# amirkdv/biseqt

Measured on AMD Instinct MI355X. Metric: GCUPS (DP cell updates/s) banded local align, higher is better.
Workload: dtype i16

## Files before the change

biseqt_amd/batch.py:

```python
import ctypes as C

import numpy as np

from . import _pwlib as W
from .sequence import Sequence

RESULT_DTYPE = np.dtype([('score', '<f8'), ('opt_i', '<i4'), ('opt_j', '<i4'),
                         ('origin_idx', '<i4'), ('mutant_idx', '<i4'),
                         ('tx_len', '<i4'), ('status', '<i4')])
assert RESULT_DTYPE.itemsize == 32
SUMMARY_DTYPE = np.dtype([(f, '<i4') for f in ('n_match', 'n_subst', 'n_ins', 'n_del', 'n_gaps', 'first_match', 'last_match',
                                               'head_origin', 'head_mutant', 'tail_origin', 'tail_mutant', 'flags')])
assert SUMMARY_DTYPE.itemsize == 48
CIGAR_EXTENDED, CIGAR_CLASSIC = W.PW_CIGAR_EXTENDED, W.PW_CIGAR_CLASSIC
CIGAR_OPS = 'MIDNSHP=X'
_CIGAR_FORMS = {'extended': CIGAR_EXTENDED, 'classic': CIGAR_CLASSIC}
SITE_DTYPE = np.dtype([('depth', '<u4'), ('call', 'u1'), ('ref', 'u1'), ('flags', '<u2')])
assert SITE_DTYPE.itemsize == 8
POLISH_STATS_DTYPE = np.dtype([(f, '<u4') for f in ('kept', 'substituted', 'deleted', 'inserted')])
assert POLISH_STATS_DTYPE.itemsize == 16
_SIDES = {'origin': W.PW_SIDE_ORIGIN, 'mutant': W.PW_SIDE_MUTANT, 'both': W.PW_SIDE_BOTH}
_CIGAR_LETTERS = ({'M': '=', 'S': 'X', 'I': 'I', 'D': 'D'}, {'M': 'M', 'S': 'M', 'I': 'I', 'D': 'D'})


# ... 742 lines not shown

def transcript_of_cigar(s):
    import re
    if not re.fullmatch(r'(?:[0-9]+[A-Za-z=])*', s):
        raise ValueError('not a CIGAR string: %r' % (s,))
    back = {'=': 'M', 'X': 'S', 'I': 'I', 'D': 'D'}
    out = []
    for n, op in re.findall(r'([0-9]+)([A-Za-z=])', s):
        if op not in back:
            raise ValueError('CIGAR op %r has no transcript letter (only the extended form =, X, I, D has)' % (op,))
        out.append(back[op] * int(n))
    return ''.join(out)


def plan_only(shapes, alnmode=W.STD_MODE, alntype=W.GLOBAL, alphabet_len=4, subst_scores=None, match_score=1, mismatch_score=0,
              go_score=0, ge_score=0, flags=0, ramp_free=False, stamp_group=False, lds_feed=False, pair_keys=False):
    lib = W.load()
    L = alphabet_len
    if subst_scores is None:
        subst_scores = [[match_score if i == j else mismatch_score for i in range(L)] for j in range(L)]
    S = np.ascontiguousarray(np.asarray(subst_scores, dtype=np.float64).reshape(L, L))
    sc = W.pw_scoring(alnmode, alntype, L, S.ctypes.data_as(C.POINTER(C.c_double)), float(go_score), float(ge_score))
    pairs = (W.pw_pair * max(len(shapes), 1))()
    off = 0
    for k, sh in enumerate(shapes):
        X, Y = int(sh[0]), int(sh[1])
        dmin, dmax = (int(sh[2]), int(sh[3])) if len(sh) > 2 else (0, 0)
        oo = off
        off += (X + 15) // 16 * 16 + 16
        mo = off
        off += (Y + 15) // 16 * 16 + 16
        pairs[k] = W.pw_pair(oo, mo, X, Y, dmin, dmax)
    name = C.create_string_buffer(128)
    info = (C.c_int32 * 8)()
    if lib.pw_plan_only(C.byref(sc), len(shapes), pairs, max(off, 16), flags, name, 128, info) != 0:
        raise RuntimeError('pw_plan_only failed: ' + W.last_error())
    out = dict(kernel=name.value.decode(), score_dtype='f64' if info[0] else 'i32', scale_shift=info[1], one_wavefront=info[2],
                workgroup=info[3], tiled=info[4], strips=info[5], packed_rule=info[6], matrix=bool(info[7] & 1))
    if ramp_free:
        out['ramp_free'] = bool(info[7] & 2)
    if stamp_group:
        out['stamp_group'] = 4 if info[7] & 4 else 1
    if lds_feed:
        out['lds_feed'] = bool(info[7] & 8)
    if pair_keys:
        out['pair_keys'] = bool(info[7] & 16)
    return out
```

biseqt_amd/csrc/build.py:

```python
import concurrent.futures
import os
import shutil
import subprocess
import sys

HERE = os.path.dirname(os.path.abspath(__file__))
ROOT = os.path.dirname(os.path.dirname(HERE))
OUT_DIR = os.path.join(os.path.dirname(HERE), 'pwlib')
OBJ_DIR = os.path.join(HERE, os.environ.get('PW_OBJ_DIR', '_build'))
SO = os.path.join(OUT_DIR, os.environ.get('PW_SO_NAME', 'pwlib.so'))
HIPCC = os.environ.get('HIPCC', '/opt/rocm/bin/hipcc')
ARCH = 'gfx950'
COMMON = ['--offload-arch=' + ARCH, '-O3', '-std=c++17', '-fPIC', '-ffp-contract=off', '-Wall',
          '-Wno-unused-function'] + os.environ.get('PW_EXTRA_CXXFLAGS', '').split()
BKS = (2, 4, 8, 16, 32)
PACKED_BKS = (4, 8, 12, 16, 20, 24, 28, 32)
PACKED_RULES = (0, 1, 2, 3, 4, 5)
PACKED_MAT_RULES = (0, 1, 2, 3)
FILL16_WAVES = {
    (8, 0, 0): (5, 0), (8, 3, 0): (5, 0),
    (16, 0, 0): (3, 0), (16, 3, 0): (3, 0),
    (8, 0, 1): (3, 0), (8, 3, 1): (3, 0),
}
for _e in filter(None, os.environ.get('PW_FILL16_WAVES_OVERRIDE', '').split(';')):
    _k, _v = _e.split('=')
    FILL16_WAVES[tuple(int(x) for x in _k.split(','))] = tuple(int(x) for x in _v.split(','))
FILL16_UNR = {}
for _e in filter(None, os.environ.get('PW_FILL16_UNR_OVERRIDE', '').split(';')):
    _k, _v = _e.split('=')
    FILL16_UNR[tuple(int(x) for x in _k.split(','))] = int(_v)
TYPES = (('i32', 'int32_t'), ('f64', 'double'))
F64_FLAGS = {'f64': ['-fno-honor-nans'] + os.environ.get('PW_F64_EXTRA_CXXFLAGS', '').split()}
FILL_EXTRA = {('f64', 8): ['-mllvm', '-amdgpu-sched-strategy=max-ilp']}
HASHED_OBJECTS = ('pw_fill16_bk8_r3_mat.o', 'pw_fill16g_bk8_r3_mat.o', 'pw_fill16l_bk8_r3_mat.o', 'pw_fill16p_bk8_r3_mat.o', 'pw_fill16_bk8_r3.o', 'pw_fill16_bk8_r0.o', 'pw_fill_i32_bk8.o', 'pw_fill_f64_bk8.o', 'pw_strip.o')
HEADERS = ['pw_types.h', 'pw_wave.h', 'pw_strip.h', 'pw_plan.h', 'pw_model.h', 'pw_launch.h', 'pw_device.h', 'pw_hip_host.h']


def _jobs():
    jobs = []
    for tn, t in TYPES:
        for bk in BKS:
            obj = os.path.join(OBJ_DIR, 'pw_fill_%s_bk%d.o' % (tn, bk))
            cmd = [HIPCC] + COMMON + F64_FLAGS.get(tn, []) + FILL_EXTRA.get((tn, bk), []) + ['-DPW_T=' + t, '-DPW_TNAME=' + tn, '-DPW_BK=%d' % bk, '-c',
                                      os.path.join(HERE, 'pw_fill_tu.hip'), '-o', obj]
            jobs.append((obj, cmd, [os.path.join(HERE, 'pw_fill_tu.hip')]))
    for tn, t in TYPES:
        obj = os.path.join(OBJ_DIR, 'pw_fill_mw_%s.o' % tn)
        cmd = [HIPCC] + COMMON + F64_FLAGS.get(tn, []) + ['-DPW_T=' + t, '-DPW_TNAME=' + tn, '-c', os.path.join(HERE, 'pw_fill_mw_tu.hip'), '-o', obj]
        jobs.append((obj, cmd, [os.path.join(HERE, 'pw_fill_mw_tu.hip')]))
# ... 10 lines not shown
               os.path.join(HERE, 'pw_fill16_tu.hip'), '-o', obj]
        jobs.append((obj, cmd, [os.path.join(HERE, 'pw_fill16_tu.hip')]))
    obj = os.path.join(OBJ_DIR, 'pw_fill16g_bk8_r3_mat.o')
    occ, occ_seg = FILL16_WAVES.get((8, 3, 1), (0, 0)) if os.environ.get('PW_FILL16_OCCUPANCY', '1') != '0' else (0, 0)
    jobs.append((obj, [HIPCC] + COMMON + ['-mllvm', '-amdgpu-sched-strategy=max-ilp', '-DPW_FILL16_WAVES=%d' % occ,
                                          '-DPW_FILL16_WAVES_SEG=%d' % occ_seg, '-c', os.path.join(HERE, 'pw_fill16g_tu.hip'), '-o', obj],
                 [os.path.join(HERE, 'pw_fill16g_tu.hip')]))
    obj = os.path.join(OBJ_DIR, 'pw_fill16l_bk8_r3_mat.o')
    jobs.append((obj, [HIPCC] + COMMON + ['-mllvm', '-amdgpu-sched-strategy=max-ilp', '-DPW_FILL16_WAVES=%d' % occ,
                                          '-DPW_FILL16_WAVES_SEG=%d' % occ_seg, '-c', os.path.join(HERE, 'pw_fill16l_tu.hip'), '-o', obj],
                 [os.path.join(HERE, 'pw_fill16l_tu.hip')]))
    obj = os.path.join(OBJ_DIR, 'pw_fill16p_bk8_r3_mat.o')
    jobs.append((obj, [HIPCC] + COMMON + ['-mllvm', '-amdgpu-sched-strategy=max-ilp', '-DPW_FILL16_WAVES=%d' % occ,
                                          '-DPW_FILL16_WAVES_SEG=%d' % occ_seg, '-c', os.path.join(HERE, 'pw_fill16p_tu.hip'), '-o', obj],
                 [os.path.join(HERE, 'pw_fill16p_tu.hip')]))
    obj = os.path.join(OBJ_DIR, 'pw_trace.o')
    jobs.append((obj, [HIPCC] + COMMON + ['-c', os.path.join(HERE, 'pw_trace.hip'), '-o', obj],
                 [os.path.join(HERE, 'pw_trace.hip')]))
    obj = os.path.join(OBJ_DIR, 'pw_txsum.o')
    jobs.append((obj, [HIPCC] + COMMON + ['-c', os.path.join(HERE, 'pw_txsum.hip'), '-o', obj],
                 [os.path.join(HERE, 'pw_txsum.hip'), os.path.join(ROOT, 'include', 'pw_txsum.h'), os.path.join(ROOT, 'include', 'pw_batch.h')]))
    obj = os.path.join(OBJ_DIR, 'pw_cigar.o')
    jobs.append((obj, [HIPCC] + COMMON + ['-c', os.path.join(HERE, 'pw_cigar.hip'), '-o', obj],
                 [os.path.join(HERE, 'pw_cigar.hip'), os.path.join(ROOT, 'include', 'pw_cigar.h'), os.path.join(ROOT, 'include', 'pw_batch.h')]))
    obj = os.path.join(OBJ_DIR, 'pw_pileup.o')
    jobs.append((obj, [HIPCC] + COMMON + ['-c', os.path.join(HERE, 'pw_pileup.hip'), '-o', obj],
                 [os.path.join(HERE, 'pw_pileup.hip'), os.path.join(ROOT, 'include', 'pw_pileup.h'), os.path.join(ROOT, 'include', 'pw_batch.h')]))
    obj = os.path.join(OBJ_DIR, 'pw_polish.o')
    jobs.append((obj, [HIPCC] + COMMON + ['-Wno-unused-parameter', '-c', os.path.join(HERE, 'pw_polish.hip'), '-o', obj],
                 [os.path.join(HERE, 'pw_polish.hip'), os.path.join(ROOT, 'include', 'pw_polish.h'), os.path.join(ROOT, 'include', 'pw_pileup.h'),
# ... 119 lines not shown
```

biseqt_amd/csrc/pw_device.h:

```cpp
#ifndef PW_DEVICE_H
#define PW_DEVICE_H

#include <hip/hip_runtime.h>
#include <stdint.h>

#define PW_FN __device__ __forceinline__
#include "pw_wave.h"
#include "pw_launch.h"

namespace pw {

PW_FN uint32_t dev_shl1_in(uint32_t m, bool flag) {
  const uint64_t mask = __builtin_amdgcn_ballot_w64(flag);
  uint32_t r;
  uint64_t cout;
  asm("v_addc_co_u32 %0, %1, %2, %2, %3" : "=v"(r), "=s"(cout) : "v"(m), "s"(mask));
  return r;
}

template <typename T, bool ALWAYS_LDS> PW_FN T dev_tab_read(const T* tab, uint32_t handle, uint32_t off, bool in_lds) {
  typedef __attribute__((address_space(3))) const T lds_T;
  if (ALWAYS_LDS || in_lds) return *(lds_T*)(uintptr_t)(handle + off);
  return *(const T*)((const char*)tab + off);
}
// ... 7 lines not shown
}

typedef uint64_t FeedDwords __attribute__((aligned(4)));
PW_FN uint64_t dev_const_dword2(const uint8_t* base, uint32_t byte_off) {
  typedef const __attribute__((address_space(4))) uint8_t c_u8;
  typedef const __attribute__((address_space(4))) FeedDwords c_fd;
  return *(c_fd*)((c_u8*)base + byte_off + 4u);
}

struct DevFeed {
  PW_FN static uint64_t const_dword2(const uint8_t* base, uint32_t byte_off) { return dev_const_dword2(base, byte_off); }
  PW_FN static uint32_t lds_read32(uint32_t addr) { return *(__attribute__((address_space(3))) const uint32_t*)(uintptr_t)addr; }
  PW_FN static void lds_write32(uint32_t addr, uint32_t v) { *(__attribute__((address_space(3))) uint32_t*)(uintptr_t)addr = v; }
  PW_FN static void lds_write16(uint32_t addr, uint32_t v) { *(__attribute__((address_space(3))) uint16_t*)(uintptr_t)addr = (uint16_t)v; }
  PW_FN static void lds_sync() { __syncthreads(); }
};

struct DevP : DevFeed {
  PW_FN static uint32_t const_dword(const uint8_t* base, int idx) { return dev_const_dword(base, idx); }
  template <typename T, bool A> PW_FN static T tab_read(const T* tab, uint32_t h, uint32_t off, bool in_lds) { return dev_tab_read<T, A>(tab, h, off, in_lds); }
  PW_FN static uint32_t shl1_in(uint32_t m, bool flag) { return dev_shl1_in(m, flag); }
  PW_FN static int lane() { return (int)(threadIdx.x & 63u); }
  PW_FN static int32_t shr1(int32_t v, int32_t old) {
    return __builtin_amdgcn_update_dpp(old, v, 0x138 , 0xf, 0xf, false);
  }
  PW_FN static int32_t shl1(int32_t v, int32_t old) {
    return __builtin_amdgcn_update_dpp(old, v, 0x130 , 0xf, 0xf, false);
  }
  PW_FN static int32_t shr1z(int32_t v) { return __builtin_amdgcn_update_dpp(0, v, 0x138 , 0xf, 0xf, true); }
  PW_FN static int32_t shl1z(int32_t v) { return __builtin_amdgcn_update_dpp(0, v, 0x130 , 0xf, 0xf, true); }
// ... 150 lines not shown
void k_fill16l(const FillParams<int32_t> a) {
  using W = WaveFill16<DevP, BK, SEG, RULE, MAT, 4, true>;
  __shared__ uint32_t ring[2 * W::kRingWords];
  const WaveDesc wd = a.waves[blockIdx.x];
  W w(a, wd);
  w.ring_h = dev_lds_handle(ring);
  w.run();
}

template <int BK, bool SEG, int RULE, bool MAT = false>
__global__ __launch_bounds__(64) PW_FILL_ATTR
__attribute__((amdgpu_waves_per_eu(Fill16Occupancy<BK, SEG, RULE>::lo, Fill16Occupancy<BK, SEG, RULE>::hi)))
void k_fill16p(const FillParams<int32_t> a) {
  using W = WaveFill16<DevP, BK, SEG, RULE, MAT, 4, true, true>;
  __shared__ uint32_t ring[2 * W::kRingWords];
  const WaveDesc wd = a.waves[blockIdx.x];
  W w(a, wd);
  w.ring_h = dev_lds_handle(ring);
  w.run();
}

template <int BK, int RULE, bool MAT = false>
__global__ __launch_bounds__(512) void k_fill16_mw(const FillParams<int32_t> a) {
  const WaveDesc wd = a.waves[blockIdx.x];
  WaveFill16<DevPM, BK, false, RULE, MAT> w(a, wd);
  w.run();
}

constexpr int kTileLanes = PW_TILE_LANES, kTileGhost = PW_TILE_GHOST, kTileCentral = kTileLanes - 2 * kTileGhost;
struct DevPT : DevFeed {
// ... 191 lines not shown
```

biseqt_amd/csrc/pw_launch.h:

```cpp
#ifndef PW_LAUNCH_H
#define PW_LAUNCH_H

#include <hip/hip_runtime_api.h>

#include "pw_plan.h"
#include "pw_types.h"

namespace pw {

hipError_t launch_fill(const FillParams<int32_t>& a, int variant, int bk, int nblocks, hipStream_t st);
hipError_t launch_fill(const FillParams<double>& a, int variant, int bk, int nblocks, hipStream_t st);
hipError_t launch_fill16(const FillParams<int32_t>& a, int bk, int seg, int rule, int mat, int nwaves, hipStream_t st);
hipError_t launch_fill16_mw(const FillParams<int32_t>& a, int bk, int rule, int mat, int nw, int npairs, hipStream_t st);
hipError_t launch_fill16g(const FillParams<int32_t>& a, int nwaves, hipStream_t st);
hipError_t launch_fill16l(const FillParams<int32_t>& a, int nwaves, hipStream_t st);
hipError_t launch_fill16p(const FillParams<int32_t>& a, int nwaves, hipStream_t st);
hipError_t launch_fill_mw(const FillParams<int32_t>& a, int variant, int bk, int nw, int nblocks, hipStream_t st);
hipError_t launch_fill_mw(const FillParams<double>& a, int variant, int bk, int nw, int nblocks, hipStream_t st);
hipError_t launch_tile(const FillParams<int32_t>& a, int variant, int pair, int ntiles, hipStream_t st);
hipError_t launch_tile(const FillParams<double>& a, int variant, int pair, int ntiles, hipStream_t st);
hipError_t launch_tile_finish(const FillParams<int32_t>& a, int pair, hipStream_t st);
hipError_t launch_tile_finish(const FillParams<double>& a, int pair, hipStream_t st);
hipError_t launch_trace(const TraceParams& p, hipStream_t st);
hipError_t launch_tx_pack(const PairDesc* pairs, const Result* results, const uint8_t* slots, int n, uint64_t* offsets,
                          uint8_t* packed, hipStream_t st);
hipError_t launch_tx_summary(const PairDesc* pairs, const Result* results, const uint8_t* slots, int n, void* out, hipStream_t st);
hipError_t launch_tx_summary_packed(const uint8_t* ops, const uint64_t* offsets, int n, void* out, hipStream_t st);
hipError_t launch_cigar_count(const PairDesc* pairs, const Result* results, const uint8_t* slots, int n, int form, uint64_t* offsets,
                              hipStream_t st);
hipError_t launch_cigar_write(const PairDesc* pairs, const Result* results, const uint8_t* slots, int n, int form, const uint64_t* offsets,
                              uint32_t* runs, hipStream_t st);
// ... 31 lines not shown
```

biseqt_amd/csrc/pw_plan.h:

```cpp
#ifndef PW_PLAN_H
#define PW_PLAN_H

#include <math.h>
#include <stdint.h>
#include <stdlib.h>

#include <algorithm>

#include "pw_model.h"
#include "pw_types.h"

namespace pw {

struct Plan {
  int rc;
  int clamped;
  int dmin, dmax;
  int num_rows;
  int64_t cells;
  int ndiag;
  int s0, nblocks, steady_b0, steady_b1;
  int brule, endrule;
};

// ... 158 lines not shown
  bool no_packed_mat = false;
  bool no_packed_anchored = false;
  bool no_packed_overlap = false;
  bool no_packed_mw = false;
  bool no_strip = false;
  bool no_small_strip = false;
  bool strip_no_byte_rows = false;
  bool no_small_tiled = false;
  bool mw_wide_lanes = false;
  int simple_as_matrix = -1;
  bool no_scaled16 = false;
  bool ramp_blocks = false;
  bool stamp_group1 = false;
  bool no_lds_feed = false;
  bool no_pair_keys = false;
  bool packed_bk_forced = false;
  int packed_bk = 0;
  bool packed_bk_seg = false;
};

static inline int packed_rule(int brule, int endrule) {
  const bool local_end = endrule == END_STD_LOCAL || endrule == END_BANDED_LOCAL;
  const bool overlap_end = endrule == END_BANDED_OVERLAP || endrule == END_STD_OVERLAP;
  if (brule == BRULE_ANY) return local_end ? 0 : endrule == END_CORNER ? 4 : -1;
  if (brule == BRULE_ORIGIN) return endrule == END_STD_LOCAL ? 5 : endrule == END_STD_OVERLAP ? 1 : endrule == END_CORNER ? 2 : -1;
  if (brule == BRULE_EDGE) return overlap_end || endrule == END_CORNER ? 1 : -1;
  return -1;
}

static inline bool packed_matrix_bytes_ok(const ScoreSummary& s, int L, bool x4) {
// ... 51 lines not shown
  return (rule == 0 || rule == 3) && matrix && !kn.ramp_blocks && ge < 0 && ge + go < 0 && smin < 0;
}

static inline int stamp_group(int rule, bool matrix, int bk, bool seg, int nw, bool ramp_free_on, const PlanKnobs& kn) {
  return (rule == 3 && matrix && bk == 8 && !seg && nw == 1 && ramp_free_on && !kn.stamp_group1) ? 4 : 1;
}

static inline bool lds_feed(int stamp_group_, const PlanKnobs& kn) { return stamp_group_ == 4 && !kn.no_lds_feed; }

static inline bool pair_keys(bool lds_feed_, const double* subst, int L, double go, double ge, const PlanKnobs& kn) {
  if (!lds_feed_ || kn.no_pair_keys || !(ge < 0) || !(go <= 0)) return false;
  for (int i = 0; i < L * L; i++)
    if (subst[i] == 0) return false;
  return true;
}

struct PackedLayout { int bk = 0, nl = 0, seg = 0, nw = 1; };

static inline PackedLayout packed_workgroup_layout(int maxnd) {
  PackedLayout l;
  l.bk = narrowest_bk(maxnd, kPackedBK, kNumPackedBK, kMaxWavesPerPair);
  if (l.bk) { l.nw = (maxnd + 64 * l.bk - 1) / (64 * l.bk); l.nl = 64 * l.nw; }
  return l;
}

static inline PackedLayout packed_lane_layout(int maxnd, int64_t sumnd, int nsolv, bool latency_mode, bool strips_win,
                                              const PlanKnobs& kn, const PlanModel& model) {
  const bool forced = kn.packed_bk_forced;
  const double meannd = (double)sumnd / nsolv;
  double cost1 = 1e300, costp = 1e300; int bk1 = 0, bkp = 0, nlp = 0;
// ... 73 lines not shown
```

biseqt_amd/csrc/pw_trace.hip:

```cpp
#include "pw_device.h"

#include <stdlib.h>

namespace pw {

__global__ __launch_bounds__(64) void k_trace(const TraceParams p, const int walkers) {
  __shared__ uint32_t win[64][WIN_WORDS + 1];
  const int pair = (int)blockIdx.x * walkers + (int)threadIdx.x;
  if ((int)threadIdx.x < walkers && pair < p.npairs) trace_walk(p, pair, win[threadIdx.x]);
}

__device__ inline uint32_t bytes_equal(uint32_t w, uint32_t c4) {
  const uint32_t v = w ^ c4;
  const uint32_t t = (v & 0x7f7f7f7fu) + 0x7f7f7f7fu;
  return ~(t | v | 0x7f7f7f7fu);
}
__global__ __launch_bounds__(64) void k_trace_fixup(const TraceParams p) {
  const int pair = (int)blockIdx.x;
  const PairDesc& pd = p.pairs[pair];
  if (!pd.solvable) return;
  const Result r = p.results[pair];
  if (!(r.status & ST_TRACED) || r.tx_len <= 0) return;
  const uint8_t* oseq = p.arena + pd.o_off;
  const uint8_t* mseq = p.arena + pd.m_off;
// ... 168 lines not shown
  return launch_fill16g_bk8_r3_m1(a, nwaves, st);
}

hipError_t launch_fill16l_bk8_r3_m1(const FillParams<int32_t>&, int, hipStream_t);
hipError_t launch_fill16l(const FillParams<int32_t>& a, int nwaves, hipStream_t st) {
  if (!a.ramp_free) return hipErrorInvalidValue;
  return launch_fill16l_bk8_r3_m1(a, nwaves, st);
}

hipError_t launch_fill16p_bk8_r3_m1(const FillParams<int32_t>&, int, hipStream_t);
hipError_t launch_fill16p(const FillParams<int32_t>& a, int nwaves, hipStream_t st) {
  if (!a.ramp_free) return hipErrorInvalidValue;
  return launch_fill16p_bk8_r3_m1(a, nwaves, st);
}

hipError_t launch_fill16_mw(const FillParams<int32_t>& a, int bk, int rule, int mat, int nw, int npairs, hipStream_t st) {
#define PW_CASE16(BK, R, MT) case ((BK) * 8 + (R)) * 2 + (MT): return launch_fill16mw_bk##BK##_r##R##_m##MT(a, nw, npairs, st);
  switch ((bk * 8 + rule) * 2 + (mat ? 1 : 0)) {
    PW_ALL16(PW_CASE16)
    default: return hipErrorInvalidValue;
  }
#undef PW_CASE16
}

hipError_t launch_fill(const FillParams<int32_t>& a, int variant, int bk, int nblocks, hipStream_t st) {
  switch (bk) {
    case 2: return launch_fill_i32_bk2(a, variant, nblocks, st);
    case 4: return launch_fill_i32_bk4(a, variant, nblocks, st);
    case 8: return launch_fill_i32_bk8(a, variant, nblocks, st);
    case 16: return launch_fill_i32_bk16(a, variant, nblocks, st);
// ... 17 lines not shown
```

biseqt_amd/csrc/pw_wave.h:

```cpp
#ifndef PW_WAVE_H
#define PW_WAVE_H

#ifndef PW_FN
#error "PW_FN must be defined by the includer"
#endif

#include "pw_types.h"
#if !defined(__HIPCC__)
#include <stdlib.h>
#endif

namespace pw {

template <typename T> struct ScoreTraits;
template <> struct ScoreTraits<int32_t> {
  static constexpr bool is_int = true;
  PW_FN static int32_t neg() { return -(1 << 28); }
  PW_FN static int32_t zero_blk() { return 0; }
  PW_FN static int32_t max2(int32_t a, int32_t b) { return a > b ? a : b; }
  PW_FN static int32_t gap_offer(bool kept, int32_t go, int32_t A) { return kept ? A : A + go; }
};
template <> struct ScoreTraits<double> {
  static constexpr bool is_int = false;
  PW_FN static double neg() { return -1.0e300; }
// ... 618 lines not shown
}
namespace pk {
inline unsigned& feed_breaches() { static unsigned n = 0; return n; }
inline unsigned* feed_path_counts() { static unsigned n[4] = {0, 0, 0, 0}; return n; }
}
extern "C" __attribute__((used, visibility("default"))) inline unsigned pw_feed_breaches(int reset) {
  const unsigned n = pk::feed_breaches();
  if (reset) pk::feed_breaches() = 0;
  return n;
}
extern "C" __attribute__((used, visibility("default"))) inline void pw_feed_path_counts(unsigned* out, int reset) {
  for (int i = 0; i < 4; i++) { out[i] = pk::feed_path_counts()[i]; if (reset) pk::feed_path_counts()[i] = 0; }
}
#endif

template <class P, int BK, bool SEG, int RULE = 0, bool MAT = false, int GRP = 1, bool LDSF = false, bool PAIRK = false>
struct WaveFill16 {
  static constexpr bool SC4 = RULE == 3;
  static constexpr int RL = SC4 ? 0 : RULE;
  static constexpr int SCL = SC4 ? 4 : 1;
  static constexpr bool ANYB = RL == 0 || RL == 4;
  static constexpr bool TRK = RL == 0 || RL == 5;
  static constexpr bool CAP = !TRK;
  static_assert(BK % 4 == 0, "packed layout needs an even number of cells per step");
  static constexpr int R = BK / 2;
  static constexpr int RH = R / 2;
#ifdef PW_FILL16_UNR
  static constexpr int UNR = PW_FILL16_UNR;
#else
  static constexpr int UNR = BK <= 8 ? 4 : (BK <= 16 ? 2 : 1);
#endif
// ... 110 lines not shown
#endif
    const int u = u0 + P::lane();
    const uint32_t row = (uint32_t)(fe + u) < (uint32_t)X ? row_of(nx_o) : 0u;
    const uint32_t code = MSEL | (((uint32_t)(ff - 256 + u) < (uint32_t)Y ? nx_m : MOUT) + 4u * sel4_fed(u));
    ring_put(0, (uint32_t)u, row, -1);
    ring_put(1, (uint32_t)u, code, 0);
    ring_put(1, (uint32_t)u + 2u, code, 1);
  }
  PW_FN void ring_begin() {
#pragma unroll 1
    for (int c = 0; c < 6; c++) { stage_issue(64 * c); stage_commit(64 * c); }
    ring_sync();
    stage_issue(384);
    ro = 4u * (uint32_t)li; rm = 4u * (uint32_t)(64 - li);
  }
  PW_FN void restage(int s) {
    stage_commit(64 * s + 384);
    ring_sync();
    stage_issue(64 * s + 448);
  }
  static constexpr bool FROWS = MAT && !SEG && UNR == 4 && BK <= 8;
  uint32_t frow[FROWS ? 8 : 1];
  bool rf;
  uint32_t flimx, flimy;
  uint32_t mrowb;
  uint8_t* mbase[BK / 4];

  PW_FN WaveFill16(const FillParams<int32_t>& a_, const WaveDesc& wd_) : a(a_), wd(wd_) {}

  template <int EK>
// ... 62 lines not shown
    uint32_t key = grp4() ? pk::mad(hk, C8, POS[k]) : pk::mad(hk, SC4 ? C2 : C8, pk::both(7 - k));
    if (EK & 2) key &= ~pk::sign(pk::sub(tl, tv), SH15);
    kb = pk::maxu(kb, key);
  }
  PW_FN void track_pair(uint32_t& kb, uint32_t H0, uint32_t H, int k) {
    kb = pk::maxu(kb, pk::mad(pk::max(H0, H), C8, POS[(k >> 1) & 3]));
  }

  template <int EK, int HALF>
  PW_FN void iteration16(int it, int k) {
    constexpr bool EDGE = EK != 0;
    const uint32_t tv0 = pk::both(2 * it), tv1 = pk::both(2 * it + 1);
    {
      uint32_t prev = up_prev;
      if (SEG) prev = segfirst ? NEGV : prev;
      const uint32_t up0 = pk::align16(UO[RH - 1], prev);
#pragma unroll
      for (int p = 0; p < RH; p++)
      {
        const uint32_t h0 = HE[p];
        cellpair<EK>(HE[p], UE[p], LE[p], bestE[p], btE[p], gebE[p], tfE[p], tlE[p], HALF == 0 ? accE[p] : acc2E[p],
                     p == 0 ? up0 : UO[p == 0 ? 0 : p - 1], LO[p], MAT ? ROW[MAT ? p : 0] : OW[p], MW[p], tv0, clE[p],
                     MAT ? ROW[MAT ? p + RH : 0] : 0u, FIXSEL && sel4_lo(k, p));
        if (TRK) {
          if (pairk()) { if (k & 1) track_pair(kbE[p], h0, HE[p], k); }
          else track_key<EK>(kbE[p], HE[p], tlE[p], tv0, k);
        }
      }
    }
    PW_IF_LDSF {
      left_next = (uint32_t)P::shl1((int32_t)LE[0], (int32_t)left_next);
      const uint32_t nxt = ring_read(0, ro, 3 + k);
#pragma unroll
      for (int i = 0; i + 1 < (MAT ? R : 1); i++) ROW[i] = ROW[i + 1];
      ROW[MAT ? R - 1 : 0] = nxt;
    } else {
      const int oi = xfeed_o + it;
      const uint32_t fb = Base::feed_byte(fo_lo, fo_hi, k);
      uint32_t feed = (!EDGE || (uint32_t)oi < (uint32_t)X) ? fb : SENT_O;
      if (MAT) feed = FROWS ? frow[FROWS ? k : 0] : row_of(fb);
      int32_t mv[2] = {(int32_t)(MAT ? ROW[0] : OW[0]), (int32_t)LE[0]};
      const int32_t mo[2] = {(int32_t)feed, (int32_t)left_next};
      xshlv<P, 2>(mv, mo, phase_l); phase_l ^= 1;
      uint32_t nxt = (uint32_t)mv[0];
      left_next = (uint32_t)mv[1];
      if (SEG) nxt = seglast ? feed : nxt;
      if (MAT) {
#pragma unroll
        for (int i = 0; i + 1 < (MAT ? R : 1); i++) ROW[i] = ROW[i + 1];
        ROW[MAT ? R - 1 : 0] = nxt;
      } else {
        const uint32_t last = pk::align16(nxt, OW[0]);
#pragma unroll
        for (int p = 0; p + 1 < RH; p++) OW[p] = OW[p + 1];
        OW[RH - 1] = last;
      }
    }
    {
      uint32_t nxt = left_next;
      if (SEG) nxt = seglast ? NEGV : nxt;
      const uint32_t leftl = pk::align16(nxt, LE[0]);
#pragma unroll
      for (int p = 0; p < RH; p++)
      {
        const uint32_t h0 = HO[p];
        cellpair<EK>(HO[p], UO[p], LO[p], bestO[p], btO[p], gebO[p], tfO[p], tlO[p], HALF == 0 ? accO[p] : acc2O[p],
                     UE[p], p == RH - 1 ? leftl : LE[p == RH - 1 ? p : p + 1], MAT ? ROW[MAT ? p : 0] : OW[p], MW[p], tv1, clO[p],
                     MAT ? ROW[MAT ? p + RH : 0] : 0u, FIXSEL && sel4_lo(k, p));
        if (TRK) {
          if (pairk()) { if (k & 1) track_pair(kbO[p], h0, HO[p], k); }
          else track_key<EK>(kbO[p], HO[p], tlO[p], tv1, k);
        }
      }
    }
    PW_IF_LDSF {
      up_prev = (uint32_t)P::shr1((int32_t)UO[RH - 1], (int32_t)up_prev);
      const uint32_t first = ring_read(1, rm, k);
#pragma unroll
      for (int p = RH - 1; p > 0; p--) MW[p] = MW[p - 1];
      MW[0] = first;
    } else {
      const int mi = yfeed_m + it;
      const uint32_t fbm = Base::feed_byte(fm_lo, fm_hi, k);
      const uint32_t feed = (MAT ? (MSEL | (fbm + 4u * (FIXSEL ? sel4_fed(k) : 1u)))
                                 : ((!EDGE || (uint32_t)mi < (uint32_t)Y) ? fbm : SENT_M)) << 16;
      int32_t mv[2] = {(int32_t)MW[RH - 1], (int32_t)UO[RH - 1]};
      const int32_t mo[2] = {(int32_t)feed, (int32_t)up_prev};
      xshrv<P, 2>(mv, mo, phase_r); phase_r ^= 1;
      uint32_t prv = (uint32_t)mv[0];
      up_prev = (uint32_t)mv[1];
      if (SEG) prv = segfirst ? feed : prv;
// ... 312 lines not shown
    mspare = (uint32_t)mask_word_index(BK, pd.nl, pd.nblocks, 0, 0);
    const bool mrow_ok = valid && li < pd.nl;
    mrow0 = mrow_ok ? (uint32_t)mask_word_index(BK, pd.nl, 0, li, 0) : mspare;
    mrow_step = mrow_ok ? (uint32_t)mask_word_index(BK, pd.nl, 1, 0, 0) : 0u;
    mrowb = 4u * mrow0;
    if (SBASE) {
#pragma unroll
      for (int g = 0; g < BK / 4; g++)
        mbase[g] = pk::opaque_s((uint8_t*)(a.masks + pd.mask_off) + (uint64_t)(4u * (uint32_t)g * mgroup));
    }
#if !defined(__HIPCC__)
    ldsf_rt = LOK && rf && P::nwaves() == 1 && pk::lds_feed_emu() == 1;
#endif
    PW_IF_LDSF { fe = e; ff = f; ring_begin(); }
    else feed_issue<true>(0);
    if constexpr (SPLIT) {
      const int nb = nblocks_run();
      const int b0 = wd.steady_b0 < nb ? (wd.steady_b0 > 0 ? wd.steady_b0 : 0) : nb;
      const int b1 = sb1 < nb ? sb1 : nb;
      const int r0 = (RAMPF && rf) ? 0 : b0, r1 = (RAMPF && rf) ? nb : b1;
      flimx = (uint32_t)(X > 7 ? X - 7 : 0); flimy = (uint32_t)(Y > 7 ? Y - 7 : 0);
      int b = 0;
      if (GRP != 4) {
        if (sb1 > wd.steady_b0) for (; b < r0; b++) blocks_step<1>(b);
        else for (; b < r0; b++) blocks_step<3>(b);
      }
      for (; b < r1; b++) blocks_step<0>(b);
      if (GRP != 4) for (; b < nb; b++) blocks_step<2>(b);
      if (grp4() && (nb & 3) != 0 && nb > 0) stamp_group((uint32_t)(nb >> 2) + 1u);
    } else {
// ... 139 lines not shown
      if (seg == sidx && li == 0) {
        Result r;
        r.score = (double)rs * a.score_mul;
        r.opt_i = a.banded ? rx - ry - pd.dmin : rx;
        r.opt_j = a.banded ? (rx < ry ? rx : ry) : ry;
        r.origin_idx = 0; r.mutant_idx = 0; r.tx_len = 0; r.status = 0;
        if (!hv || (endrule == END_STD_LOCAL && !(rs > 0))) { r.opt_i = -1; r.opt_j = -1; r.score = 0.0; }
        a.results[pair_slot] = r;
      }
    }
  }
  uint32_t ring_h = 0;
  uint32_t ro, rm;
  uint32_t nx_o, nx_m;
  int fe, ff;
#if !defined(__HIPCC__)
  bool pairk_rt = false;
#endif
};
#undef PW_IF_LDSF

PW_FN int pw_first_op(uint32_t mask) {
  return (mask & 1u) ? 0 : (mask & 2u) ? 1 : (mask & 4u) ? 2 : 3;
}


enum { WIN_B = 4, WIN_WORDS = WIN_B * 2 * 4 };

PW_FN void trace_walk(const TraceParams& p, int pair, uint32_t* win ) {
  const PairDesc pdv = p.pairs[pair];
// ... 99 lines not shown
```

biseqt_amd/csrc/pwlib_api.cpp:

```cpp
#include <hip/hip_runtime.h>
#include <math.h>
#include <cmath>
#include <stdint.h>
#include <stdio.h>
#include <stdlib.h>
#include <string.h>

#include <algorithm>
#include <string>
#include <chrono>
#include <memory>
#include <mutex>
#include <thread>
#include <vector>
#include <unordered_set>

#include "../../include/pw_batch.h"
#include "../../include/pw_txsum.h"
#include "../../include/pw_cigar.h"
#include "../../include/pw_pileup.h"
#include "../../include/pw_polish.h"
#include "../../include/pw_graph.h"
#include "../../include/pw_consensus.h"
#include "pw_launch.h"
// ... 160 lines not shown
  std::vector<pw::WaveDesc> waves;
  std::vector<int32_t> strips;
  std::vector<uint32_t> strip_ctl_init;
  PoolBuffer<uint64_t> d_fifo; size_t fifo_bytes = 0;
  DeviceArray<pw::StripBest> d_sbest;
  DeviceArray<uint32_t> d_ctl;
  std::vector<int32_t> tiled;
  DeviceBuffer d_state[2];
  int32_t st_pitch = 0;
  int packed_seg = 0, packed_rule = 0, packed_nw = 1;
  int packed_mat = 0;
  int ramp_free = 0;
  int stamp_group = 1;
  int lds_feed = 0;
  int pair_keys = 0;
  DeviceArray<pw::WaveDesc> d_waves;
  int64_t cells = 0, alg_bytes = 0;
  bool on_device = false;
  PoolBuffer<uint8_t> arena; uint64_t arena_bytes = 0;
  uint8_t* d_arena = nullptr;
  bool arena_shared = false;
  PoolBuffer<pw::PairDesc> d_pairs;
  PoolBuffer<uint32_t> d_masks; uint64_t mask_words = 0;
  DeviceBuffer d_hdump; uint64_t h_elems = 0;
  PoolBuffer<pw::Result> d_results;
  PoolBuffer<uint8_t> d_tx; uint64_t tx_bytes = 0;
  DeviceBuffer d_subst;
  DeviceArray<int32_t> d_ends;
  PoolBuffer<uint8_t> d_txpacked;
  DeviceArray<uint64_t> d_txoffsets;
// ... 37 lines not shown
  k.no_packed_mat = on("PWLIB_NO_PACKED_MAT");
  k.no_packed_anchored = on("PWLIB_NO_PACKED_ANCHORED");
  k.no_packed_overlap = on("PWLIB_NO_PACKED_OVERLAP");
  k.no_packed_mw = on("PWLIB_NO_PACKED_MW");
  k.no_strip = on("PWLIB_NO_STRIP");
  k.no_small_strip = on("PWLIB_NO_SMALL_STRIP");
  k.strip_no_byte_rows = on("PWLIB_STRIP_NO_BYTE_ROWS");
  k.no_small_tiled = on("PWLIB_NO_SMALL_TILED");
  k.mw_wide_lanes = on("PWLIB_MW_WIDE_LANES");
  k.simple_as_matrix = env_int("PWLIB_SIMPLE_AS_MATRIX", -1);
  k.no_scaled16 = on("PWLIB_NO_SCALED16");
  k.ramp_blocks = on("PWLIB_RAMP_BLOCKS");
  k.stamp_group1 = env_int("PWLIB_STAMP_GROUP", 0) == 1;
  k.no_lds_feed = env_int("PWLIB_LDS_FEED", 1) == 0;
  k.no_pair_keys = env_int("PWLIB_PAIR_KEYS", 1) == 0;
  const char* bk = getenv("PWLIB_PACKED_BK");
  if (bk && *bk) { k.packed_bk_forced = true; k.packed_bk = atoi(bk); k.packed_bk_seg = strchr(bk, 's') != nullptr; }
  return k;
}

int batch_inputs(pw_batch* b, bool plan_only, const pw_scoring* sc, int32_t n_pairs, const pw_pair* pairs, uint64_t arena_bytes,
                 uint32_t flags) {
  if (!sc || n_pairs < 0 || (n_pairs > 0 && !pairs) || (plan_only && !sc->subst))
    return fail(plan_only ? "pw_plan_only: bad arguments" : "pw_batch_create: bad arguments");
  if (sc->mode != pw::STD_MODE && sc->mode != pw::BANDED_MODE) return fail("unknown alignment mode");
  if (sc->type < 0 || sc->type > (sc->mode == pw::STD_MODE ? 6 : 2)) return fail("unknown alignment type");
  if (sc->alphabet_len < 1 || sc->alphabet_len > 256 || !sc->subst) return fail("alphabet_len must be 1..256 with a score matrix");
  b->n = n_pairs; b->flags = flags;
  b->mode = sc->mode; b->type = sc->type; b->L = sc->alphabet_len; b->go = sc->go; b->ge = sc->ge;
  b->subst.assign(sc->subst, sc->subst + (size_t)b->L * b->L);
// ... 107 lines not shown
    if (maxnd > 2048) {
      if (maxnd <= 64 * pw::kMaxWavesPerPair * 32 && !kn.no_packed_mw && !strips_win) p16 = pw::packed_workgroup_layout(maxnd);
    } else {
      p16 = pw::packed_lane_layout(maxnd, sumnd, nsolv, latency_mode, strips_win, kn, model);
    }
  }
  if (p16.bk) {
    b->variant = pw::VAR_FAST16;
    b->packed_seg = p16.seg; b->packed_nw = p16.nw;
    b->packed_mat = pw::packed_matrix_form(adm, p16, sc.simple, kn);
    b->packed_rule = adm.x4 && (!b->packed_mat || adm.x4_matrix) ? 3 : adm.rule;
    b->ramp_free = pw::ramp_free(b->packed_rule, b->packed_mat != 0, b->go, b->ge, sc.smin, kn);
    b->stamp_group = pw::stamp_group(b->packed_rule, b->packed_mat != 0, p16.bk, p16.seg != 0, p16.nw, b->ramp_free != 0, kn);
    b->lds_feed = pw::lds_feed(b->stamp_group, kn) ? 1 : 0;
    b->pair_keys = pw::pair_keys(b->lds_feed != 0, b->subst.data(), L, b->go, b->ge, kn) ? 1 : 0;
  }
  pw::PairRules pr;
  pr.strips = strips_serve && !b->use_f64 && b->variant != pw::VAR_GENERIC && b->variant != pw::VAR_FAST16 &&
              !(b->flags & PW_FLAG_FORCE_TILED);
  pr.all_strips = (b->flags & PW_FLAG_FORCE_STRIP) != 0;
  pr.few_strips = latency_mode && !kn.no_small_strip && est.strips_beat_workgroups(model);
  pr.all_tiled = (b->flags & PW_FLAG_FORCE_TILED) != 0;
  pr.few_tiled = latency_mode && !(b->flags & PW_FLAG_DUMP_SCORES) && !kn.no_small_tiled && est.tiles_beat_workgroups(model, b->use_f64);
  pr.latency_mode = latency_mode; pr.f64 = b->use_f64; pr.wide_lanes = kn.mw_wide_lanes;
  pr.packed_bk = p16.bk; pr.packed_nl = p16.nl;
  for (int32_t k = 0; k < b->n; k++) {
    pw::PairDesc& d = b->descs[k];
    if (!d.solvable) continue;
    const pw::PairLayout lay = pw::pair_layout(d.ndiag, d.X, pr);
    d.bk = lay.bk; d.nl = lay.nl;
// ... 205 lines not shown
      HIP_TRY(pw::launch_tile(a, b->variant, (int)k, ntiles, st));
      cur ^= 1;
    }
    a.st_in = b->d_state[cur].as<const T>();
    HIP_TRY(pw::launch_tile_finish(a, (int)k, st));
  }
  return 0;
}

int launch_packed_fill(pw_batch* b, hipStream_t st) {
  pw::FillParams<int32_t> a = fill_params<int32_t>(b);
  a.order = b->classes[0].d_order.p; a.waves = b->d_waves.p;
  if (b->packed_mat) pw::packed_matrix_rows(b->subst.data(), b->L, b->packed_rule == 3, a.mat_rows, &a.mat_bias);
  a.ramp_free = b->ramp_free;
  if (b->packed_nw > 1) HIP_TRY(pw::launch_fill16_mw(a, b->classes[0].bk, b->packed_rule, b->packed_mat, b->packed_nw, (int)b->waves.size(), st));
  else if (b->pair_keys) HIP_TRY(pw::launch_fill16p(a, (int)b->waves.size(), st));
  else if (b->lds_feed) HIP_TRY(pw::launch_fill16l(a, (int)b->waves.size(), st));
  else if (b->stamp_group == 4) HIP_TRY(pw::launch_fill16g(a, (int)b->waves.size(), st));
  else HIP_TRY(pw::launch_fill16(a, b->classes[0].bk, b->packed_seg, b->packed_rule, b->packed_mat, (int)b->waves.size(), st));
  return 0;
}

}

extern "C" {

const char* pw_last_error(void) { return g_err.c_str(); }

void pw_pool_trim(void) { pool_drop(-1); }

// ... 23 lines not shown
}

void pw_batch_destroy(pw_batch* b) { delete b; }

int pw_plan_only(const pw_scoring* sc, int32_t n_pairs, const pw_pair* pairs, uint64_t arena_bytes, uint32_t flags,
                 char* kernel, int32_t kernel_cap, int32_t* info) {
  pw_batch b;
  b.device = -1;
  if (batch_inputs(&b, true, sc, n_pairs, pairs, arena_bytes, flags) != 0 || batch_plan(&b) != 0) return -1;
  if (kernel && kernel_cap > 0) { strncpy(kernel, pw_batch_kernel_name(&b), (size_t)kernel_cap - 1); kernel[kernel_cap - 1] = 0; }
  if (info) {
    int64_t one = 0, wg = 0;
    for (const auto& c : b.classes) (c.nw > 1 || (b.variant == pw::VAR_FAST16 && b.packed_nw > 1) ? wg : one) += (int64_t)c.order.size();
    info[0] = b.use_f64 ? 1 : 0; info[1] = b.scale_shift; info[2] = (int32_t)one; info[3] = (int32_t)wg;
    info[4] = (int32_t)b.tiled.size(); info[5] = (int32_t)b.strips.size();
    info[6] = b.variant == pw::VAR_FAST16 ? b.packed_rule : -1; info[7] = (b.packed_mat ? 1 : 0) | (b.ramp_free ? 2 : 0) | (b.stamp_group == 4 ? 4 : 0) | (b.lds_feed ? 8 : 0) | (b.pair_keys ? 16 : 0);
  }
  return 0;
}

int pw_batch_init_rc(const pw_batch* b, int32_t k) { return (k < 0 || k >= b->n) ? -1 : b->plans[k].rc; }

int pw_batch_band(const pw_batch* b, int32_t k, int32_t* dmin, int32_t* dmax, int32_t* num_rows) {
  if (k < 0 || k >= b->n) return -1;
  if (dmin) *dmin = b->plans[k].dmin;
  if (dmax) *dmax = b->plans[k].dmax;
  if (num_rows) *num_rows = b->plans[k].num_rows;
  return b->plans[k].clamped;
}

int64_t pw_batch_pair_cells(const pw_batch* b, int32_t k) { return (k < 0 || k >= b->n) ? -1 : b->plans[k].cells; }
// ... 1248 lines not shown
```

Baseline: 3183.

## Exchange neighbour boundary values through LDS instead of cross-lane shifts

Adds a new fill16 kernel variant (fill16x) where the up and left boundary values between adjacent lanes are written as 16-bit halves into an LDS offer buffer and read back as 32-bit words. This replaces the cross-lane shift (shr1/shl1) and align16 sequence. It is selected by default whenever pair_keys is active. The aim is to take DPP/permute work off the serial dependency chain, at the cost of more LDS traffic and reliance on write-to-read ordering within a wavefront.

```diff
diff --git a/biseqt_amd/batch.py b/biseqt_amd/batch.py
--- a/biseqt_amd/batch.py
+++ b/biseqt_amd/batch.py
@@ -780,7 +780,8 @@
 
 
 def plan_only(shapes, alnmode=W.STD_MODE, alntype=W.GLOBAL, alphabet_len=4, subst_scores=None, match_score=1, mismatch_score=0,
-              go_score=0, ge_score=0, flags=0, ramp_free=False, stamp_group=False, lds_feed=False, pair_keys=False):
+              go_score=0, ge_score=0, flags=0, ramp_free=False, stamp_group=False, lds_feed=False, pair_keys=False,
+              lds_exchange=False):
     lib = W.load()
     L = alphabet_len
     if subst_scores is None:
@@ -811,4 +812,6 @@
         out['lds_feed'] = bool(info[7] & 8)
     if pair_keys:
         out['pair_keys'] = bool(info[7] & 16)
+    if lds_exchange:
+        out['lds_exchange'] = bool(info[7] & 32)
     return out
diff --git a/biseqt_amd/csrc/build.py b/biseqt_amd/csrc/build.py
--- a/biseqt_amd/csrc/build.py
+++ b/biseqt_amd/csrc/build.py
@@ -32,7 +32,7 @@
 TYPES = (('i32', 'int32_t'), ('f64', 'double'))
 F64_FLAGS = {'f64': ['-fno-honor-nans'] + os.environ.get('PW_F64_EXTRA_CXXFLAGS', '').split()}
 FILL_EXTRA = {('f64', 8): ['-mllvm', '-amdgpu-sched-strategy=max-ilp']}
-HASHED_OBJECTS = ('pw_fill16_bk8_r3_mat.o', 'pw_fill16g_bk8_r3_mat.o', 'pw_fill16l_bk8_r3_mat.o', 'pw_fill16p_bk8_r3_mat.o', 'pw_fill16_bk8_r3.o', 'pw_fill16_bk8_r0.o', 'pw_fill_i32_bk8.o', 'pw_fill_f64_bk8.o', 'pw_strip.o')
+HASHED_OBJECTS = ('pw_fill16_bk8_r3_mat.o', 'pw_fill16g_bk8_r3_mat.o', 'pw_fill16l_bk8_r3_mat.o', 'pw_fill16p_bk8_r3_mat.o', 'pw_fill16x_bk8_r3_mat.o', 'pw_fill16_bk8_r3.o', 'pw_fill16_bk8_r0.o', 'pw_fill_i32_bk8.o', 'pw_fill_f64_bk8.o', 'pw_strip.o')
 HEADERS = ['pw_types.h', 'pw_wave.h', 'pw_strip.h', 'pw_plan.h', 'pw_model.h', 'pw_launch.h', 'pw_device.h', 'pw_hip_host.h']
 
 
@@ -73,6 +73,11 @@
     jobs.append((obj, [HIPCC] + COMMON + ['-mllvm', '-amdgpu-sched-strategy=max-ilp', '-DPW_FILL16_WAVES=%d' % occ,
                                           '-DPW_FILL16_WAVES_SEG=%d' % occ_seg, '-c', os.path.join(HERE, 'pw_fill16p_tu.hip'), '-o', obj],
                  [os.path.join(HERE, 'pw_fill16p_tu.hip')]))
+    obj = os.path.join(OBJ_DIR, 'pw_fill16x_bk8_r3_mat.o')
+    dirs = ['-DPW_FILL16X_DIRS=' + os.environ['PW_FILL16X_DIRS']] if os.environ.get('PW_FILL16X_DIRS') else []
+    jobs.append((obj, [HIPCC] + COMMON + ['-mllvm', '-amdgpu-sched-strategy=max-ilp', '-DPW_FILL16_WAVES=%d' % occ,
+                                          '-DPW_FILL16_WAVES_SEG=%d' % occ_seg] + dirs + ['-c', os.path.join(HERE, 'pw_fill16x_tu.hip'), '-o', obj],
+                 [os.path.join(HERE, 'pw_fill16x_tu.hip')]))
     obj = os.path.join(OBJ_DIR, 'pw_trace.o')
     jobs.append((obj, [HIPCC] + COMMON + ['-c', os.path.join(HERE, 'pw_trace.hip'), '-o', obj],
                  [os.path.join(HERE, 'pw_trace.hip')]))
diff --git a/biseqt_amd/csrc/pw_device.h b/biseqt_amd/csrc/pw_device.h
--- a/biseqt_amd/csrc/pw_device.h
+++ b/biseqt_amd/csrc/pw_device.h
@@ -45,6 +45,14 @@
   PW_FN static void lds_write32(uint32_t addr, uint32_t v) { *(__attribute__((address_space(3))) uint32_t*)(uintptr_t)addr = v; }
   PW_FN static void lds_write16(uint32_t addr, uint32_t v) { *(__attribute__((address_space(3))) uint16_t*)(uintptr_t)addr = (uint16_t)v; }
   PW_FN static void lds_sync() { __syncthreads(); }
+  typedef uint16_t __attribute__((may_alias)) xch16_t;
+  typedef uint32_t __attribute__((may_alias)) xch32_t;
+  PW_FN static void lds_put_halves(uint32_t addr, uint32_t v) {
+    *(__attribute__((address_space(3))) xch16_t*)(uintptr_t)addr = (uint16_t)v;
+    *(__attribute__((address_space(3))) xch16_t*)(uintptr_t)(addr + 2u) = (uint16_t)(v >> 16);
+  }
+  PW_FN static void lds_put32(uint32_t addr, uint32_t v) { *(__attribute__((address_space(3))) xch32_t*)(uintptr_t)addr = v; }
+  PW_FN static uint32_t lds_take32(uint32_t addr) { return *(__attribute__((address_space(3))) const xch32_t*)(uintptr_t)addr; }
 };
 
 struct DevP : DevFeed {
@@ -225,6 +233,21 @@
 void k_fill16p(const FillParams<int32_t> a) {
   using W = WaveFill16<DevP, BK, SEG, RULE, MAT, 4, true, true>;
   __shared__ uint32_t ring[2 * W::kRingWords];
+  const WaveDesc wd = a.waves[blockIdx.x];
+  W w(a, wd);
+  w.ring_h = dev_lds_handle(ring);
+  w.run();
+}
+
+#ifndef PW_FILL16X_DIRS
+#define PW_FILL16X_DIRS 3
+#endif
+template <int BK, bool SEG, int RULE, bool MAT = false>
+__global__ __launch_bounds__(64) PW_FILL_ATTR
+__attribute__((amdgpu_waves_per_eu(Fill16Occupancy<BK, SEG, RULE>::lo, Fill16Occupancy<BK, SEG, RULE>::hi)))
+void k_fill16x(const FillParams<int32_t> a) {
+  using W = WaveFill16<DevP, BK, SEG, RULE, MAT, 4, true, true, PW_FILL16X_DIRS>;
+  __shared__ uint32_t ring[2 * W::kRingWords + 2 * kOfferWords];
   const WaveDesc wd = a.waves[blockIdx.x];
   W w(a, wd);
   w.ring_h = dev_lds_handle(ring);
diff --git a/biseqt_amd/csrc/pw_fill16x_tu.hip b/biseqt_amd/csrc/pw_fill16x_tu.hip
--- /dev/null
+++ b/biseqt_amd/csrc/pw_fill16x_tu.hip
@@ -0,0 +1,8 @@
+#include "pw_device.h"
+
+namespace pw {
+hipError_t launch_fill16x_bk8_r3_m1(const FillParams<int32_t>& a, int nwaves, hipStream_t st) {
+  hipLaunchKernelGGL((k_fill16x<8, false, 3, true>), dim3((unsigned)nwaves), dim3(64), 0, st, a);
+  return hipGetLastError();
+}
+}
diff --git a/biseqt_amd/csrc/pw_launch.h b/biseqt_amd/csrc/pw_launch.h
--- a/biseqt_amd/csrc/pw_launch.h
+++ b/biseqt_amd/csrc/pw_launch.h
@@ -15,6 +15,7 @@
 hipError_t launch_fill16g(const FillParams<int32_t>& a, int nwaves, hipStream_t st);
 hipError_t launch_fill16l(const FillParams<int32_t>& a, int nwaves, hipStream_t st);
 hipError_t launch_fill16p(const FillParams<int32_t>& a, int nwaves, hipStream_t st);
+hipError_t launch_fill16x(const FillParams<int32_t>& a, int nwaves, hipStream_t st);
 hipError_t launch_fill_mw(const FillParams<int32_t>& a, int variant, int bk, int nw, int nblocks, hipStream_t st);
 hipError_t launch_fill_mw(const FillParams<double>& a, int variant, int bk, int nw, int nblocks, hipStream_t st);
 hipError_t launch_tile(const FillParams<int32_t>& a, int variant, int pair, int ntiles, hipStream_t st);
diff --git a/biseqt_amd/csrc/pw_plan.h b/biseqt_amd/csrc/pw_plan.h
--- a/biseqt_amd/csrc/pw_plan.h
+++ b/biseqt_amd/csrc/pw_plan.h
@@ -196,6 +196,7 @@
   bool stamp_group1 = false;
   bool no_lds_feed = false;
   bool no_pair_keys = false;
+  bool no_lds_exchange = false;
   bool packed_bk_forced = false;
   int packed_bk = 0;
   bool packed_bk_seg = false;
@@ -277,6 +278,8 @@
     if (subst[i] == 0) return false;
   return true;
 }
+
+static inline bool lds_exchange(bool pair_keys_, const PlanKnobs& kn) { return pair_keys_ && !kn.no_lds_exchange; }
 
 struct PackedLayout { int bk = 0, nl = 0, seg = 0, nw = 1; };
 
diff --git a/biseqt_amd/csrc/pw_trace.hip b/biseqt_amd/csrc/pw_trace.hip
--- a/biseqt_amd/csrc/pw_trace.hip
+++ b/biseqt_amd/csrc/pw_trace.hip
@@ -206,6 +206,12 @@
   return launch_fill16p_bk8_r3_m1(a, nwaves, st);
 }
 
+hipError_t launch_fill16x_bk8_r3_m1(const FillParams<int32_t>&, int, hipStream_t);
+hipError_t launch_fill16x(const FillParams<int32_t>& a, int nwaves, hipStream_t st) {
+  if (!a.ramp_free) return hipErrorInvalidValue;
+  return launch_fill16x_bk8_r3_m1(a, nwaves, st);
+}
+
 hipError_t launch_fill16_mw(const FillParams<int32_t>& a, int bk, int rule, int mat, int nw, int npairs, hipStream_t st) {
 #define PW_CASE16(BK, R, MT) case ((BK) * 8 + (R)) * 2 + (MT): return launch_fill16mw_bk##BK##_r##R##_m##MT(a, nw, npairs, st);
   switch ((bk * 8 + rule) * 2 + (mat ? 1 : 0)) {
diff --git a/biseqt_amd/csrc/pw_wave.h b/biseqt_amd/csrc/pw_wave.h
--- a/biseqt_amd/csrc/pw_wave.h
+++ b/biseqt_amd/csrc/pw_wave.h
@@ -656,7 +656,34 @@
 }
 #endif
 
-template <class P, int BK, bool SEG, int RULE = 0, bool MAT = false, int GRP = 1, bool LDSF = false, bool PAIRK = false>
+static constexpr uint32_t kOfferWords = 65, kOfferLeft = 4u * kOfferWords;
+template <class P, bool LDS, bool TAKE>
+PW_FN uint32_t offer_up(uint32_t xa, uint32_t& carried, uint32_t own) {
+  if constexpr (LDS) {
+    if (TAKE) return P::lds_take32(xa);
+    P::lds_put_halves(xa + 2u, own);
+    return 0u;
+  } else {
+    if (TAKE) return pk::align16(own, carried);
+    carried = (uint32_t)P::shr1((int32_t)own, (int32_t)carried);
+    return 0u;
+  }
+}
+template <class P, bool LDS, bool TAKE>
+PW_FN uint32_t offer_left(uint32_t xa, uint32_t& carried, uint32_t own) {
+  if constexpr (LDS) {
+    if (TAKE) return P::lds_take32(xa + kOfferLeft + 4u);
+    P::lds_put_halves(xa + kOfferLeft + 2u, own);
+    return 0u;
+  } else {
+    if (TAKE) return pk::align16(carried, own);
+    carried = (uint32_t)P::shl1((int32_t)own, (int32_t)carried);
+    return 0u;
+  }
+}
+
+template <class P, int BK, bool SEG, int RULE = 0, bool MAT = false, int GRP = 1, bool LDSF = false, bool PAIRK = false,
+          int XLDS = 0>
 struct WaveFill16 {
   static constexpr bool SC4 = RULE == 3;
   static constexpr int RL = SC4 ? 0 : RULE;
@@ -797,6 +824,15 @@
     stage_issue(384);
     ro = 4u * (uint32_t)li; rm = 4u * (uint32_t)(64 - li);
   }
+  static constexpr bool XUP = (XLDS & 1) != 0, XLEFT = (XLDS & 2) != 0;
+  static_assert(XLDS == 0 || (LDSF && XLDS <= 3), "offers through LDS: the form of the kernel that reads its letters from LDS");
+  PW_FN void offers_begin() {
+    if constexpr (XLDS != 0) {
+      xch_a = ring_h + 4u * (uint32_t)(2 * kRingWords) + 4u * (uint32_t)P::lane();
+      if (XUP) { P::lds_put32(xch_a, up_prev >> 16); offer_up<P, true, false>(xch_a, up_prev, UO[RH - 1]); }
+      if (XLEFT) P::lds_put32(xch_a + kOfferLeft + 4u, left_next << 16);
+    }
+  }
   PW_FN void restage(int s) {
     stage_commit(64 * s + 384);
     ring_sync();
@@ -889,7 +925,7 @@
     {
       uint32_t prev = up_prev;
       if (SEG) prev = segfirst ? NEGV : prev;
-      const uint32_t up0 = pk::align16(UO[RH - 1], prev);
+      const uint32_t up0 = offer_up<P, XUP, true>(xch_a, prev, UO[RH - 1]);
 #pragma unroll
       for (int p = 0; p < RH; p++)
       {
@@ -904,7 +940,7 @@
       }
     }
     PW_IF_LDSF {
-      left_next = (uint32_t)P::shl1((int32_t)LE[0], (int32_t)left_next);
+      offer_left<P, XLEFT, false>(xch_a, left_next, LE[0]);
       const uint32_t nxt = ring_read(0, ro, 3 + k);
 #pragma unroll
       for (int i = 0; i + 1 < (MAT ? R : 1); i++) ROW[i] = ROW[i + 1];
@@ -934,7 +970,7 @@
     {
       uint32_t nxt = left_next;
       if (SEG) nxt = seglast ? NEGV : nxt;
-      const uint32_t leftl = pk::align16(nxt, LE[0]);
+      const uint32_t leftl = offer_left<P, XLEFT, true>(xch_a, nxt, LE[0]);
 #pragma unroll
       for (int p = 0; p < RH; p++)
       {
@@ -949,7 +985,7 @@
       }
     }
     PW_IF_LDSF {
-      up_prev = (uint32_t)P::shr1((int32_t)UO[RH - 1], (int32_t)up_prev);
+      offer_up<P, XUP, false>(xch_a, up_prev, UO[RH - 1]);
       const uint32_t first = ring_read(1, rm, k);
 #pragma unroll
       for (int p = RH - 1; p > 0; p--) MW[p] = MW[p - 1];
@@ -1292,6 +1328,7 @@
 #endif
     PW_IF_LDSF { fe = e; ff = f; ring_begin(); }
     else feed_issue<true>(0);
+    if constexpr (XLDS != 0) offers_begin();
     if constexpr (SPLIT) {
       const int nb = nblocks_run();
       const int b0 = wd.steady_b0 < nb ? (wd.steady_b0 > 0 ? wd.steady_b0 : 0) : nb;
@@ -1461,6 +1498,7 @@
   uint32_t ro, rm;
   uint32_t nx_o, nx_m;
   int fe, ff;
+  uint32_t xch_a = 0;
 #if !defined(__HIPCC__)
   bool pairk_rt = false;
 #endif
diff --git a/biseqt_amd/csrc/pwlib_api.cpp b/biseqt_amd/csrc/pwlib_api.cpp
--- a/biseqt_amd/csrc/pwlib_api.cpp
+++ b/biseqt_amd/csrc/pwlib_api.cpp
@@ -198,6 +198,7 @@
   int stamp_group = 1;
   int lds_feed = 0;
   int pair_keys = 0;
+  int lds_exchange = 0;
   DeviceArray<pw::WaveDesc> d_waves;
   int64_t cells = 0, alg_bytes = 0;
   bool on_device = false;
@@ -265,6 +266,7 @@
   k.stamp_group1 = env_int("PWLIB_STAMP_GROUP", 0) == 1;
   k.no_lds_feed = env_int("PWLIB_LDS_FEED", 1) == 0;
   k.no_pair_keys = env_int("PWLIB_PAIR_KEYS", 1) == 0;
+  k.no_lds_exchange = env_int("PWLIB_LDS_EXCHANGE", 1) == 0;
   const char* bk = getenv("PWLIB_PACKED_BK");
   if (bk && *bk) { k.packed_bk_forced = true; k.packed_bk = atoi(bk); k.packed_bk_seg = strchr(bk, 's') != nullptr; }
   return k;
@@ -402,6 +404,7 @@
     b->stamp_group = pw::stamp_group(b->packed_rule, b->packed_mat != 0, p16.bk, p16.seg != 0, p16.nw, b->ramp_free != 0, kn);
     b->lds_feed = pw::lds_feed(b->stamp_group, kn) ? 1 : 0;
     b->pair_keys = pw::pair_keys(b->lds_feed != 0, b->subst.data(), L, b->go, b->ge, kn) ? 1 : 0;
+    b->lds_exchange = pw::lds_exchange(b->pair_keys != 0, kn) ? 1 : 0;
   }
   pw::PairRules pr;
   pr.strips = strips_serve && !b->use_f64 && b->variant != pw::VAR_GENERIC && b->variant != pw::VAR_FAST16 &&
@@ -637,6 +640,7 @@
   if (b->packed_mat) pw::packed_matrix_rows(b->subst.data(), b->L, b->packed_rule == 3, a.mat_rows, &a.mat_bias);
   a.ramp_free = b->ramp_free;
   if (b->packed_nw > 1) HIP_TRY(pw::launch_fill16_mw(a, b->classes[0].bk, b->packed_rule, b->packed_mat, b->packed_nw, (int)b->waves.size(), st));
+  else if (b->lds_exchange) HIP_TRY(pw::launch_fill16x(a, (int)b->waves.size(), st));
   else if (b->pair_keys) HIP_TRY(pw::launch_fill16p(a, (int)b->waves.size(), st));
   else if (b->lds_feed) HIP_TRY(pw::launch_fill16l(a, (int)b->waves.size(), st));
   else if (b->stamp_group == 4) HIP_TRY(pw::launch_fill16g(a, (int)b->waves.size(), st));
@@ -690,7 +694,7 @@
     for (const auto& c : b.classes) (c.nw > 1 || (b.variant == pw::VAR_FAST16 && b.packed_nw > 1) ? wg : one) += (int64_t)c.order.size();
     info[0] = b.use_f64 ? 1 : 0; info[1] = b.scale_shift; info[2] = (int32_t)one; info[3] = (int32_t)wg;
     info[4] = (int32_t)b.tiled.size(); info[5] = (int32_t)b.strips.size();
-    info[6] = b.variant == pw::VAR_FAST16 ? b.packed_rule : -1; info[7] = (b.packed_mat ? 1 : 0) | (b.ramp_free ? 2 : 0) | (b.stamp_group == 4 ? 4 : 0) | (b.lds_feed ? 8 : 0) | (b.pair_keys ? 16 : 0);
+    info[6] = b.variant == pw::VAR_FAST16 ? b.packed_rule : -1; info[7] = (b.packed_mat ? 1 : 0) | (b.ramp_free ? 2 : 0) | (b.stamp_group == 4 ? 4 : 0) | (b.lds_feed ? 8 : 0) | (b.pair_keys ? 16 : 0) | (b.lds_exchange ? 32 : 0);
   }
   return 0;
 }
```

New measurement: 3295 (median of 6 runs). +3.5%, better.
